# Yongda1/Ab-initio-Flexible-Gaussian-Basis-Neural-Network-Quantum-Monte-Carlo

Hardware: AMD Instinct MI355X
Metric: walker·steps/sec + local-energy evals/sec, N2 14e⁻ 4096 walkers, 1/2/4/8 MI355X (higher is better)
Workload: dtype f32

## Files before the change

### ab-initio-flexible-gaussian-basis-neural-network-quantum-monte-carlo_amd/csrc/quad_small.h

```cpp
#pragma once
#include "walker_rev.h"

namespace aq {

template <typename T> __device__ __forceinline__ T row16_sum(T x) {
  x += dpp<0x128>(x);
  x += dpp<0x124>(x);
  x += dpp<0x122>(x);
  x += dpp<0x121>(x);
  return x;
}
template <typename T> __device__ __forceinline__ T row_class4_sum(T x) {
  x += dpp<0x124>(x);
  x += dpp<0x128>(x);
  return x;
}

template <int N> struct QSlot {
  static constexpr int SW = N <= 4 ? 16 : 32;
  static constexpr int NI = SW / 4;
  static constexpr int NSL = 64 / SW;
};
template <int SW, typename T> __device__ __forceinline__ T slot_sum(T x) {
  x = row16_sum(x);
// ... 524 lines not shown
        if (acc && act) {
#pragma unroll
          for (int c = 0; c < 3; ++c) ((T*)ka.pos)[(size_t)conf * 3 * N + 3 * sl + c] = xn[c];
          if (ka.acc.count) atomicAdd(&ka.acc.count[conf], 1);
        }
      }
    } else if (sl < 3 * N) {
      xs[sl] = ((const T*)ka.pos)[(size_t)conf * 3 * N + sl];
    }
    wave_sync();
    {
      const int c = sl / NI, e = sl % NI;
      const int ee = e < N ? e : N - 1;
      const bool elive = e < N, ev = c == 3;
      ElecOut<T, A> eo;
      electron_stage<T, N, A>(P, xs + ee * 3, ee, c, eo);
      T* Wl = Wc + WC::loc + 16 * (ev ? 0 : c) + ee;
#pragma unroll
      for (int col = 0; col < N; ++col) {
        PJ<T> sy = P[Ly::wy + col] * eo.yst[0];
#pragma unroll
        for (int m = 1; m < NYW; ++m) sy = sy + P[Ly::wy + m * N + col] * eo.yst[m];
        const PJ<T> yt = eo.env * sy;
        lv[col] = yt.d1;
        if (elive && ev) {
          Yv[e * N + col] = yt.v;
          if (act) Wc[WC::yv + e * N + col] = yt.v;
        }
        if (elive && !ev && act) Wl[col * 48] = yt.d1;
      }
#pragma unroll
      for (int m = 0; m < D0; ++m) {
        lv[N + m] = eo.hf[m].d1;
        if (elive && ev) {
          hl[e * D0 + m] = eo.hf[m].v;
          if (act) Wc[WC::h0 + e * D0 + m] = eo.hf[m].v;
        }
        if (elive && !ev && act) Wl[(N + m) * 48] = eo.hf[m].d1;
      }
      if (elive && ev) {
        jsum = eo.jae.v;
        if (act) Wc[WC::jaev + e] = eo.jae.v;
      }
      if (elive && !ev) {
        jd1w = eo.jae.d1;
        if (act) Wc[WC::jaed + 16 * c + e] = jd1w;
      }
    }
    T jl = T(0);
#pragma unroll
    for (int it0 = 0; it0 < N * N; it0 += SW) {
      const int it = it0 + sl;
      const bool pl = it < N * N;
      const int k = pl ? it / N : 0, i = pl ? it - (it / N) * N : 0;
      const bool diag = k == i;
      T d[3];
#pragma unroll
      for (int c = 0; c < 3; ++c) d[c] = xs[i * 3 + c] - xs[k * 3 + c];
      const T r2 = d[0] * d[0] + d[1] * d[1] + d[2] * d[2];
      const T r = f_sqrt(diag ? T(1) : r2);
      T pp[4] = {diag ? T(0) : r, diag ? T(0) : d[0], diag ? T(0) : d[1], diag ? T(0) : d[2]};
      if (pl && k < i) {
        const T cusp = P[Ly::jee_c + k * N + i], al = P[Ly::jee_a + k * N + i];
        jl += f_div(cusp * r, al * r + T(1));
      }
      if (pl) {
#pragma unroll
        for (int f = 0; f < 4; ++f) S[it * 12 + f] = pp[f];
      }
#pragma unroll
      for (int j = 0; j < 2; ++j) {
        const cptr<T> dw = P + (j == 0 ? Ly::dbl_w0 : Ly::dbl_w1);
        const cptr<T> db = P + (j == 0 ? Ly::dbl_b0 : Ly::dbl_b1);
        T q[4];
#pragma unroll
        for (int o = 0; o < 4; ++o) {
          T z = db[o];
#pragma unroll
          for (int m = 0; m < 4; ++m) z += pp[m] * dw[m * 4 + o];
          q[o] = f_tanh(z);
        }
        if (pl && !diag && act) {
#pragma unroll
          for (int o = 0; o < 4; ++o) Wc[WC::pt + (k * N + i) * 8 + j * 4 + o] = q[o];
        }
#pragma unroll
        for (int o = 0; o < 4; ++o) {
          pp[o] = (pp[o] + q[o]) * RSQ2;
          if (pl) S[it * 12 + (j + 1) * 4 + o] = pp[o];
        }
      }
    }
    {
      jsum += jl;
      const T jee = slot_sum<SW>(jl);
      if (sl == 0 && act) Wc[WC::jee] = jee;
    }
    wave_sync();
    for (int t = sl; t < 24 * N; t += SW) {
      const int f = t & 3, ci = (t >> 2) % N, lg = (t >> 2) / N;
      const int l = lg >> 1, G = lg & 1;
      const int k0 = G ? nup : 0, k1 = G ? N : nup;
      T acc = T(0);
      for (int k = k0; k < k1; ++k) acc += S[(k * N + ci) * 12 + l * 4 + f];
      const T v = acc * (G ? ginv1 : ginv0);
      g2[((l * 2 + G) * N + ci) * 4 + f] = v;
      if (act) Wc[WC::g2 + ((l * 2 + G) * N + ci) * 4 + f] = v;
    }
    wave_sync();
  } else {
  jsum = quad_stage_load<T, N, A, SW>((const T*)ka.pos + (size_t)pb * 3 * N, Wc, Eq, pi, sl, xs, sm + SQ::xo, Yv,
                                      hl, g2);
  wave_sync();

  {
    const int part = sl / NI, o = sl % NI;
    const int os = o < N ? o : N - 1;
    const T* xp = (part & 1) ? sm + SQ::xo : xs + pi * 3;
    T d[3];
#pragma unroll
    for (int c = 0; c < 3; ++c) d[c] = part < 2 ? xs[os * 3 + c] - xp[c] : xp[c] - xs[os * 3 + c];
    T v[3][4];
    pair_values<T, N, A>(d, P, v);
    T dv[3][4];
#pragma unroll
    for (int l = 0; l < 3; ++l)
#pragma unroll
      for (int f = 0; f < 4; ++f) dv[l][f] = v[l][f] - dpp<0x100 + NI>(v[l][f]);
    if (part < 2 && o < N && o != pi) {
      const T cusp = P[Ly::jee_c + pi * N + o], al = P[Ly::jee_a + pi * N + o];
      const T je = f_div(cusp * v[0][0], al * v[0][0] + T(1));
      jsum += part == 0 ? je : -je;
    }
    if (part == 0 && o < N && o != pi) {
      const int Gp = pi >= nup ? 1 : 0;
      const T gw = Gp ? ginv1 : ginv0;
#pragma unroll
      for (int l = 0; l < 3; ++l)
#pragma unroll
        for (int f = 0; f < 4; ++f) g2[((l * 2 + Gp) * N + o) * 4 + f] += dv[l][f] * gw;
    }
    if (part == 2) {
#pragma unroll
      for (int l = 0; l < 3; ++l)
#pragma unroll
        for (int f = 0; f < 4; ++f) S[o * 12 + l * 4 + f] = dv[l][f];
    }
  }
  wave_sync();
#pragma unroll
  for (int t0 = 0; t0 < 24; t0 += SW) {
    const int t = t0 + sl;
    if (t < 24) {
      const int l = t >> 3, G = (t >> 2) & 1, f = t & 3;
      const int k0 = G ? nup : 0, k1 = G ? N : nup;
      T acc = T(0);
      for (int k = k0; k < k1; ++k)
        if (k != pi) acc += S[k * 12 + l * 4 + f];
      g2[((l * 2 + G) * N + pi) * 4 + f] += acc * (G ? ginv1 : ginv0);
    }
  }
  wave_sync();
  }

  const int fi = sl >> 2, ff = sl & 3;
  const bool ilive = fi < N;
  const int ic = ilive ? fi : N - 1;
// ... 492 lines not shown
```

### ab-initio-flexible-gaussian-basis-neural-network-quantum-monte-carlo_amd/csrc/walker_rev.h

```cpp
#pragma once
#include "jets.h"
#include "layout.h"
#include "walker_kernel.h"
#include "gj.h"
#include "electron.h"

namespace aq {

#ifdef AQ_PHASE_PROF
static __device__ unsigned long long aq_phase_cycles[32];
#define AQ_PH(k)                                                                         \
  do {                                                                                   \
    const unsigned long long t_ = __builtin_readcyclecounter();                          \
    if (lane == 0) atomicAdd(&aq_phase_cycles[(ka.proposal ? 16 : 0) + (k)], t_ - t_ph); \
    t_ph = t_;                                                                           \
  } while (0)
#elif defined(AQ_PHASE_MARK)
#define AQ_PH(k) asm volatile(";AQMARK " #k)
#elif defined(AQ_STOP_AFTER)
#define AQ_PH(k)                                                                     \
  do {                                                                               \
    if constexpr (PROP && (k) == AQ_STOP_AFTER) {                                    \
      if (ka.logabs) ((T*)ka.logabs)[conf * 64 + lane] = sm[lane] + sm[lane + 1024]; \
      return;                                                                        \
    }                                                                                \
  } while (0)
#else
#define AQ_PH(k) \
  do {           \
  } while (0)
#endif

#ifdef AQ_ABLATE
#define AQ_ABL(b) (isprop && (ka.ablate & (b)))
#else
#define AQ_ABL(b) false
#endif

#ifndef AQ_NO_FWD_REG
constexpr bool kFwdReg = true;
#else
constexpr bool kFwdReg = false;
#endif
template <typename T, int N, int A, bool FWDREG = false, bool COMPACT = false>
struct SmemRev {
  static constexpr int D0 = 4 * A;
  static constexpr int DFM = 3 * D0 + 8;
  static constexpr int QM = DFM / 4;
  static constexpr int hl_n = N * D0 + N * 4;
  static constexpr int cmax(int a, int b) { return a > b ? a : b; }
  static constexpr int xs = 0;
  static constexpr int hl = 48;
  static constexpr int hbar = hl;
  static constexpr int QL = (3 * 4 + 8) / 4;
  static constexpr int cq = hl + hl_n;
  static constexpr int sv = cq + (FWDREG ? 0 : N * QM + 2 * N * QL);
  static constexpr int cqo(int l, int i) { return l == 0 ? i * QM : N * QM + ((l - 1) * N + i) * QL; }
  static constexpr int g2 = sv + (FWDREG ? 0 : 3 * N * 4);
  static constexpr int yv = g2 + 3 * 2 * N * 4;
  static constexpr int ybar = yv;
  static constexpr int R = yv + N * N;
  static constexpr int ph = R;
  static constexpr int mx = COMPACT ? R : R + N * N * 2;
  static constexpr int dbar = R;
  static constexpr int R_n = COMPACT ? cmax(cmax(2 * N * N, 3 * N * N), 4 + 32 * 12)
                                     : cmax(cmax(4 * N * N, 3 * N * N), 4 + 64 * 12);
  static constexpr int pv = g2;
  static constexpr int RW = (N + 3) / 4;
  static constexpr int st = ((g2 + 3 * N + 2 + 3) / 4) * 4;
  static constexpr int zr = st + (4 * RW * 4 * 4 + (int)sizeof(T) - 1) / (int)sizeof(T);
  static_assert(zr + 4 <= g2 + 3 * 2 * N * 4, "slot table outside the g2 region");
  static constexpr int jdo = R + R_n;
  static constexpr int end = jdo + (FWDREG ? 64 : 0);
  static constexpr int bytes = ((end * (int)sizeof(T)) + 15) & ~15;
  static constexpr int hoff(int l) { return l == 0 ? 0 : N * D0; }
};

template <int N, int A>
struct WCache {
  static constexpr int D0 = 4 * A;
  static constexpr int yv = 0;
  static constexpr int h0 = yv + N * N;
  static constexpr int loc = h0 + N * D0;
  static constexpr int jaev = loc + (N + D0) * 48;
  static constexpr int jaed = jaev + N;
  static constexpr int g2 = jaed + 48;
  static constexpr int jee = g2 + 3 * 2 * N * 4;
  static constexpr int pv = jee + 1;
  static constexpr int pt = ((pv + 3 * N + 2 + 3) / 4) * 4;
  static constexpr int size = ((pt + 8 * N * N + 63) / 64) * 64;
};
template <int N, int A>
struct ECache {
  static constexpr int D0 = 4 * A;
  static constexpr int yv = 0;
  static constexpr int h0 = N;
  static constexpr int yd = N + D0;
  static constexpr int hd = yd + 3 * N;
  static constexpr int jv = hd + 3 * D0;
  static constexpr int jd = jv + 1;
  static constexpr int xp = jd + 3;
  static constexpr int size = ((xp + 3 + 15) / 16) * 16;
};

template <typename T, int N, int A>
__device__ __forceinline__ void pair_values(const T d[3], cptr<T> P, T out[3][4]) {
  using Ly = Lay<N, A>;
  const T RSQ2 = T(0.70710678118654752);
  T p[4];
  p[0] = f_sqrt(d[0] * d[0] + d[1] * d[1] + d[2] * d[2]);
#pragma unroll
  for (int c = 0; c < 3; ++c) p[1 + c] = d[c];
#pragma unroll
  for (int f = 0; f < 4; ++f) out[0][f] = p[f];
#pragma unroll
  for (int j = 0; j < 2; ++j) {
    const cptr<T> dw = P + (j == 0 ? Ly::dbl_w0 : Ly::dbl_w1);
    const cptr<T> db = P + (j == 0 ? Ly::dbl_b0 : Ly::dbl_b1);
    T q[4];
#pragma unroll
    for (int o = 0; o < 4; ++o) {
      T s = db[o];
#pragma unroll
      for (int m = 0; m < 4; ++m) s += p[m] * dw[m * 4 + o];
      q[o] = f_tanh(s);
    }
#pragma unroll
    for (int o = 0; o < 4; ++o) {
      p[o] = (p[o] + q[o]) * RSQ2;
      out[j + 1][o] = p[o];
    }
  }
}

template <typename T> __device__ __forceinline__ T class4_sum(T x) {
  x += dpp<0x124>(x);
  x += dpp<0x128>(x);
#ifdef AQ_PERMLANE_SUM
  if constexpr (sizeof(T) == 4) {
    const auto a = __builtin_amdgcn_permlane16_swap(__float_as_uint(x), __float_as_uint(x), false, false);
    x = __uint_as_float(a[0]) + __uint_as_float(a[1]);
    const auto b = __builtin_amdgcn_permlane32_swap(__float_as_uint(x), __float_as_uint(x), false, false);
    return __uint_as_float(b[0]) + __uint_as_float(b[1]);
  }
#endif
  x += __shfl_xor(x, 16);
  x += __shfl_xor(x, 32);
  return x;
}
template <int M, typename T> __device__ __forceinline__ T quad_bcast(T x) {
  return dpp<M | (M << 2) | (M << 4) | (M << 6)>(x);
}

template <typename T, int NV, int NU>
__device__ __forceinline__ void ld_use(cptr<T> p, T* out) {
  static_assert(NU <= NV, "record");
  if constexpr (sizeof(T) == 4) {
    typedef float f4 __attribute__((ext_vector_type(4)));
    typedef float f2 __attribute__((ext_vector_type(2)));
    const __attribute__((address_space(4))) f4* q = (const __attribute__((address_space(4))) f4*)p;
#pragma unroll
    for (int j = 0; j < NU / 4; ++j) {
      const f4 v = q[j];
      out[4 * j] = v.x;
      out[4 * j + 1] = v.y;
      out[4 * j + 2] = v.z;
      out[4 * j + 3] = v.w;
    }
    constexpr int B = NU / 4 * 4, R = NU % 4;
    if constexpr (R >= 2) {
      const f2 v = *(const __attribute__((address_space(4))) f2*)(p + B);
      out[B] = v.x;
      out[B + 1] = v.y;
    }
    if constexpr (R == 1 || R == 3) out[B + R - 1] = p[B + R - 1];
#pragma unroll
    for (int k = NU; k < NV; ++k) out[k] = T(0);
  } else {
#pragma unroll
    for (int k = 0; k < NV; ++k) out[k] = k < NU ? p[k] : T(0);
  }
}

template <typename T, int NV>
__device__ __forceinline__ void ld_vec(cptr<T> p, T* out) {
  if constexpr (sizeof(T) == 4) {
    typedef float f4 __attribute__((ext_vector_type(4)));
    const __attribute__((address_space(4))) f4* q = (const __attribute__((address_space(4))) f4*)p;
#pragma unroll
    for (int j = 0; j < NV / 4; ++j) {
      const f4 v = q[j];
      out[4 * j] = v.x;
      out[4 * j + 1] = v.y;
      out[4 * j + 2] = v.z;
      out[4 * j + 3] = v.w;
    }
  } else {
    typedef double d2 __attribute__((ext_vector_type(2)));
    const __attribute__((address_space(4))) d2* q = (const __attribute__((address_space(4))) d2*)p;
#pragma unroll
    for (int j = 0; j < NV / 2; ++j) {
      const d2 v = q[j];
      out[2 * j] = v.x;
      out[2 * j + 1] = v.y;
    }
  }
}
#ifndef AQ_NO_XLANE
constexpr bool kXLane = true;
#else
constexpr bool kXLane = false;
#endif

__device__ __forceinline__ void wave_sync() {
  __builtin_amdgcn_fence(__ATOMIC_RELEASE, "wavefront");
// ... 145 lines not shown
  T* E = (T*)ka.ecache + (size_t)q0 * EC::size;
#pragma unroll
  for (int col = 0; col < N; ++col) {
    PJ<T> sy = P[Ly::wy + col] * eo.yst[0];
#pragma unroll
    for (int m = 1; m < NYW; ++m) sy = sy + P[Ly::wy + m * N + col] * eo.yst[m];
    E[EC::yv + col] = (eo.env * sy).v;
  }
#pragma unroll
  for (int m = 0; m < D0; ++m) E[EC::h0 + m] = eo.hf[m].v;
  E[EC::jv] = eo.jae.v;
#pragma unroll
  for (int c = 0; c < 3; ++c) E[EC::xp + c] = xp[c];
}

#ifndef AQ_PROP_WAVES
#define AQ_PROP_WAVES 5
#endif
#ifndef AQ_PREP_WAVES
#define AQ_PREP_WAVES 4
#endif
template <typename T, int N, int A, bool PREP, bool PROP, bool PW7 = false> struct RevWaves {
  static constexpr int value = PW7 ? 7 : (PREP ? (sizeof(T) == 4 ? AQ_PREP_WAVES : 2) : ((sizeof(T) == 4 && N == 14 && A == 2) ? (PROP ? AQ_PROP_WAVES : 4) : 1));
};

#ifndef AQ_PROP_WPB
#define AQ_PROP_WPB 2
#endif
#ifndef AQ_WALK_WPB
#define AQ_WALK_WPB 1
#endif
template <typename T, bool PROP, bool PREP = false> struct RevWpb {
  static constexpr int value = sizeof(T) != 4 ? 1 : (PROP ? AQ_PROP_WPB : (PREP ? 1 : AQ_WALK_WPB));
};
#ifdef AQ_WAVE_SYNC
#define AQ_SYNC() wave_sync()
#else
#define AQ_SYNC()                                   \
  do {                                              \
    if constexpr (WPB > 1) wave_sync();             \
    else __syncthreads();                           \
  } while (0)
#endif

template <typename T, int N, int A>
__device__ __forceinline__ void b3_pair_adjoint(cptr<T> P, const T* xs, const T* g2b, T* dbar, int nup, int k, int i,
                                                bool may_fresh, bool fresh, const T* tcache, T cusp, T al) {
  using Ly = Lay<N, A>;
  const T RSQ2 = T(0.70710678118654752);
  cptr<T> Pq = P;
  asm volatile("" : "+s"(Pq));
  const int G = k >= nup ? 1 : 0;
  T d[3];
#pragma unroll
  for (int c = 0; c < 3; ++c) d[c] = xs[i * 3 + c] - xs[k * 3 + c];
  const T r = f_sqrt(d[0] * d[0] + d[1] * d[1] + d[2] * d[2]);
  T p0[4] = {r, d[0], d[1], d[2]};
  T t1[4], t2[4];
#pragma unroll
  for (int o = 0; o < 4; ++o) {
    t1[o] = tcache ? tcache[o] : T(0);
    t2[o] = tcache ? tcache[4 + o] : T(0);
  }
  if (may_fresh) {
    T f1[4], p1[4], f2[4];
#pragma unroll
    for (int o = 0; o < 4; ++o) {
      T s = Pq[Ly::dbl_b0 + o];
#pragma unroll
      for (int m = 0; m < 4; ++m) s += p0[m] * Pq[Ly::dbl_w0 + m * 4 + o];
      f1[o] = f_tanh(s);
    }
#pragma unroll
    for (int o = 0; o < 4; ++o) p1[o] = (p0[o] + f1[o]) * RSQ2;
#pragma unroll
    for (int o = 0; o < 4; ++o) {
      T s = Pq[Ly::dbl_b1 + o];
#pragma unroll
      for (int m = 0; m < 4; ++m) s += p1[m] * Pq[Ly::dbl_w1 + m * 4 + o];
      f2[o] = f_tanh(s);
    }
#pragma unroll
    for (int o = 0; o < 4; ++o) {
      t1[o] = fresh ? f1[o] : t1[o];
      t2[o] = fresh ? f2[o] : t2[o];
    }
  }
  T pb2[4], pb1[4], pb0[4];
#pragma unroll
  for (int f = 0; f < 4; ++f) pb2[f] = g2b[((2 * 2 + G) * N + i) * 4 + f];
  T z2[4];
#pragma unroll
  for (int o = 0; o < 4; ++o) z2[o] = pb2[o] * RSQ2 * (T(1) - t2[o] * t2[o]);
#pragma unroll
  for (int m = 0; m < 4; ++m) {
    T s = g2b[((1 * 2 + G) * N + i) * 4 + m] + pb2[m] * RSQ2;
#pragma unroll
    for (int o = 0; o < 4; ++o) s += z2[o] * Pq[Ly::dbl_w1 + m * 4 + o];
    pb1[m] = s;
  }
  T z1[4];
#pragma unroll
  for (int o = 0; o < 4; ++o) z1[o] = pb1[o] * RSQ2 * (T(1) - t1[o] * t1[o]);
#pragma unroll
  for (int m = 0; m < 4; ++m) {
    T s = g2b[((0 * 2 + G) * N + i) * 4 + m] + pb1[m] * RSQ2;
#pragma unroll
    for (int o = 0; o < 4; ++o) s += z1[o] * Pq[Ly::dbl_w0 + m * 4 + o];
    pb0[m] = s;
  }
  T rb = pb0[0];
  {
    const T den = al * r + T(1);
    rb += and_zero(k < i, cusp * f_rcp(den * den));
  }
  const T ir = f_rcp(r);
#pragma unroll
  for (int c = 0; c < 3; ++c) dbar[(k * N + i) * 3 + c] = pb0[1 + c] + rb * d[c] * ir;
}

template <typename T, int N>
__device__ __forceinline__ void walker_draws(const __attribute__((address_space(4))) KArgs* kl, int conf, int lane) {
  if (kl->dg1 && lane < N) {
    const uint32_t t = (uint32_t)(conf * N + lane);
    const uint64_t seed = kl->seed, step = kl->step;
    float a[3], b[3], c[4];
    philox_normal3f(seed, step, t, 0u, a);
    philox_normal3f(seed, step, t, 1u, b);
    philox_u4(seed, step, t, 2u, c);
#pragma unroll
    for (int k = 0; k < 3; ++k) {
      ((T*)kl->dg1)[(size_t)t * 3 + k] = (T)a[k];
      ((T*)kl->dg2)[(size_t)t * 3 + k] = (T)b[k];
    }
    ((T*)kl->du)[t] = (T)(c[0] - 5.9604644775390625e-08f);
  }
}

template <typename T, int N, int A, bool PREP = false, bool PROP = false, bool PW7 = false, bool PH = false,
          bool SPL = false>
__global__ __attribute__((amdgpu_flat_work_group_size(1, 64 * (SPL ? 2 : RevWpb<T, PROP, PREP>::value)))) __attribute__((amdgpu_waves_per_eu(RevWaves<T, N, A, PREP, PROP, PW7>::value))) void
k_walker_rev(KArgs ka) {
  static_assert(!PW7 || (PROP && !PREP), "PW7 is a proposal instantiation");
  static_assert(!PH || PREP, "PH is an adjoint-pass instantiation");
  static_assert(!SPL || (!PROP && !PREP), "SPL is a walker-launch instantiation");
  using Ly = Lay<N, A>;
  constexpr bool fwd_reg = PROP && kFwdReg;
  constexpr bool compact = PROP && PW7 && fwd_reg;
  constexpr bool xlane = PROP && kXLane;
  using SM = SmemRev<T, N, A, fwd_reg, compact>;
  using LCc = LapCache<N, A>;
  constexpr int D0 = SM::D0;
  constexpr int WPB = SPL ? 2 : RevWpb<T, PROP, PREP>::value;
  const cptr<T> P = param_ptr<T>(ka.prm);
  extern __shared__ __attribute__((aligned(16))) unsigned char smem_raw[];
  const int wv = WPB > 1 ? __builtin_amdgcn_readfirstlane((int)(threadIdx.x >> 6)) : 0;
  T* sm = (T*)(smem_raw + (SPL ? 0 : wv) * SM::bytes);
  T* xs = sm + SM::xs;

  const bool isprop = PROP ? true : (ka.proposal != 0);
  const int conf = SPL ? xcd_major(blockIdx.x, gridDim.x) : xcd_major(blockIdx.x, gridDim.x) * WPB + wv;
  if (WPB > 1 && conf >= ka.nconf) return;
  const int lane = WPB > 1 ? (int)(threadIdx.x & 63) : (int)threadIdx.x;
  const int lc = lane >> 4;
  const int er = lane & 15;
  const int le = er < N ? er : N - 1;
  const bool val = (lc == 3);
  const bool live = er < N;
  const bool dir = (lc < 3) && live;
  const int nup = ka.nup;
  const T tstep = (T)ka.tstep;
  const T RSQ2 = T(0.70710678118654752);
  const T ginv0 = T(1) / T(nup), ginv1 = T(1) / T(N - nup);
  const int* rowsrc = ka.rowsrc;
#ifdef AQ_PHASE_PROF
  unsigned long long t_ph = __builtin_readcyclecounter();
#endif

  int pb = conf, pi = -1;
  if (isprop) {
    const int mper = ka.mper ? ka.mper : N, mdiv = ka.mdiv ? ka.mdiv : 1;
    pb = conf / mper;
    pi = (conf - pb * mper) / mdiv;
  }
  const T te_walk = (!PROP && isprop && !ka.xnew) ? taueff_wave<T>(ka.taueff, ka.tacc, 0, ka.tstep, ka.tpart) : T(0);
  if (SPL && wv != 0) {
  } else if (!PREP && !isprop && ka.acc.lpn) {
    const T te1 = taueff_wave<T>(ka.acc.taueff, ka.acc.tacc, 0, ka.acc.tstep, ka.acc.tpart);
    const T te2 = taueff_wave<T>(ka.acc.taueff, ka.acc.tacc, 1, ka.acc.tstep, ka.acc.tpart);
    if (lane < N) {
      T xn[3];
      const bool acc = accept_one<T, N>(ka.acc, (const T*)ka.pos, conf, lane, xn, te1, te2);
#pragma unroll
      for (int c = 0; c < 3; ++c) xs[3 * lane + c] = xn[c];
      if (acc) {
#pragma unroll
        for (int c = 0; c < 3; ++c) ((T*)ka.pos)[(size_t)conf * 3 * N + 3 * lane + c] = xn[c];
        if (ka.acc.count) atomicAdd(&ka.acc.count[conf], 1);
      }
    }
  } else if (!PROP && lane < 3 * N) {
    T x = ((const T*)ka.pos)[(size_t)pb * 3 * N + lane];
    if (isprop && lane / 3 == pi) {
      sm[SM::R + (lane - 3 * pi)] = x;
      if (ka.xnew) {
        x = ((const T*)ka.xnew)[(size_t)conf * 3 + (lane - 3 * pi)];
      } else {
        const T z = ((const T*)ka.gauss1)[(size_t)pb * 3 * N + lane];
        const T ge = ((const T*)ka.pgrad)[(size_t)pb * 3 * N + lane] * te_walk;
        x = x + (ge * tstep + f_sqrt(tstep) * z);
      }
    }
    xs[lane] = x;
  }
  if constexpr (SPL) __syncthreads();
  else if constexpr (!PROP) AQ_SYNC();

  AQ_PH(0);
  using WC = WCache<N, A>;
  using EC = ECache<N, A>;
  const bool reuse = !PREP && PROP;
#ifndef AQ_NO_F1_GLDS
  constexpr bool f1_glds = PROP;
#else
  constexpr bool f1_glds = false;
#endif
  const bool wfix = !PREP && !PROP && !isprop && ka.pvok != 0;
  T* Wc = (T*)ka.wcache + (size_t)(reuse ? pb : conf) * WC::size;
  T* Lw = PREP ? (T*)ka.lapcache + (size_t)conf * LCc::size : nullptr;
  const T* Eq = reuse ? (const T*)ka.ecache + (size_t)conf * EC::size : nullptr;
  T* Yv = sm + SM::yv;
  T* g2 = sm + SM::g2;
  T jv = T(0), jd1 = T(0), jve = T(0);
  T jsum_p = T(0);
  T pvr = T(0);
  int rsl = 0;
  T jvp = T(0);
  auto f2_pair_values = [&](T cusp, T al) {
    T* S = sm + SM::R + 4;
    const T* xo = sm + SM::R;
    const int o = lane & 15, part = lane >> 4;
    const int os = o < N ? o : N - 1;
    const T* xp = (part & 1) ? xo : xs + pi * 3;
    T d[3];
#pragma unroll
    for (int c = 0; c < 3; ++c) d[c] = (part < 2) ? xs[os * 3 + c] - xp[c] : xp[c] - xs[os * 3 + c];
    T v[3][4];
    pair_values<T, N, A>(d, P, v);
    if constexpr (compact) {
#pragma unroll
      for (int l = 0; l < 3; ++l)
#pragma unroll
        for (int f = 0; f < 4; ++f) {
          const T w = __shfl_down(v[l][f], 16);
          if ((part & 1) == 0) S[(16 * (part >> 1) + o) * 12 + l * 4 + f] = v[l][f] - w;
        }
    } else {
#pragma unroll
    for (int l = 0; l < 3; ++l)
#pragma unroll
      for (int f = 0; f < 4; ++f) S[lane * 12 + l * 4 + f] = v[l][f];
    }
    if (part < 2 && o < N && o != pi) {
      if constexpr (!PROP) {
        cusp = P[Ly::jee_c + pi * N + o];
        al = P[Ly::jee_a + pi * N + o];
      }
      const T je = f_div(cusp * v[0][0], al * v[0][0] + T(1));
      jvp += part == 0 ? je : -je;
    }
  };
  auto jee_params = [&](T& cusp, T& al) {
    const int os = (lane & 15) < N ? (lane & 15) : N - 1;
    cusp = P[Ly::jee_c + pi * N + os];
    al = P[Ly::jee_a + pi * N + os];
  };
  if (reuse) {
    constexpr int NY = (N * N + 63) / 64, NHh = (N * D0 + 63) / 64, NG = (3 * 2 * N * 4 + 63) / 64;
    T ry[NY], rh[NHh], rg[NG];
    T eyv = T(0), eh0 = T(0);
    if constexpr (f1_glds) {
      lds_dma<T>(Yv, Wc + WC::yv, N * N, lane);
      lds_dma<T>(sm + SM::hl, Wc + WC::h0, N * D0, lane);
      lds_dma<T>(g2, Wc + WC::g2, 3 * 2 * N * 4, lane);
      eyv = Eq[EC::yv + (lane < N ? lane : N - 1)];
      eh0 = Eq[EC::h0 + (lane < D0 ? lane : D0 - 1)];
    }
    const bool mvl = lane < 3 * N && lane / 3 == pi;
    T x0 = T(0), xm = T(0), jc = T(0), ja = T(0);
    if constexpr (PROP) {
      const int l3 = lane < 3 * N ? lane : 3 * N - 1;
      x0 = ((const T*)ka.pos)[(size_t)pb * 3 * N + l3];
      xm = Eq[EC::xp + (mvl ? lane - 3 * pi : 0)];
      jee_params(jc, ja);
      rsl = rowsrc[lane < N ? lane : N - 1];
    }
    if constexpr (!f1_glds) {
#pragma unroll
    for (int t = 0; t < NY; ++t) {
      const unsigned idx = lane + 64 * t;
      const unsigned ix = idx < N * N ? idx : N * N - 1;
      const unsigned r = ix / N;
      const T a = Wc[WC::yv + ix], b = Eq[EC::yv + (ix - r * N)];
      ry[t] = ((int)r == pi) ? b : a;
    }
#pragma unroll
    for (int t = 0; t < NHh; ++t) {
      const unsigned idx = lane + 64 * t;
      const unsigned ix = idx < N * D0 ? idx : N * D0 - 1;
      const unsigned e = ix / D0;
      const T a = Wc[WC::h0 + ix], b = Eq[EC::h0 + (ix - e * D0)];
      rh[t] = ((int)e == pi) ? b : a;
    }
#pragma unroll
    for (int t = 0; t < NG; ++t) {
      const int idx = lane + 64 * t;
      rg[t] = Wc[WC::g2 + (idx < 3 * 2 * N * 4 ? idx : 3 * 2 * N * 4 - 1)];
    }
    }
    {
      if constexpr (PROP) {
        const T* js = (er == pi) ? Eq + EC::jv : Wc + WC::jaev + le;
        jv = and_zero(val && live, *js);
        const T* ds = (le == pi) ? Eq + EC::jd + (lc < 3 ? lc : 0) : Wc + WC::jaed + (lane < 48 ? lane : 47);
        jd1 = and_zero(dir, *ds);
        jve = and_zero(lane == 0, Wc[WC::jee]);
      } else {
        const T a = Wc[WC::jaev + le], b = Eq[EC::jv];
        jv = (val && live) ? ((er == pi) ? b : a) : T(0);
        const T a1 = Wc[WC::jaed + (lane < 48 ? lane : 47)], b1 = Eq[EC::jd + (lc < 3 ? lc : 0)];
        jd1 = dir ? ((le == pi) ? b1 : a1) : T(0);
// ... 75 lines not shown
#pragma unroll
        for (int l = 0; l < 3; ++l)
#pragma unroll
          for (int f = 0; f < 4; ++f)
            g2[((l * 2 + Gp) * N + lane) * 4 + f] +=
                (compact ? S[lane * 12 + l * 4 + f] : S[lane * 12 + l * 4 + f] - S[(16 + lane) * 12 + l * 4 + f]) * gw;
      }
    } else if (lane < 40) {
      const int t = lane - 16;
      const int l = t >> 3, G = (t >> 2) & 1, f = t & 3;
      const int k0 = G ? nup : 0, k1 = G ? N : nup;
      T acc = T(0);
#pragma unroll
      for (int k = 0; k < N; ++k) {
        const T dv = compact ? S[(16 + k) * 12 + l * 4 + f] : S[(32 + k) * 12 + l * 4 + f] - S[(48 + k) * 12 + l * 4 + f];
        acc += (k >= k0 && k < k1 && k != pi) ? dv : T(0);
      }
      g2[((l * 2 + G) * N + pi) * 4 + f] += acc * (G ? ginv1 : ginv0);
    }
  } else if (!reuse && (!SPL || wv == 1)) {
    {
      const int i = lane >> 2, kq = lane & 3;
      const bool icol = i < N;
      const int ii = icol ? i : N - 1;
      T acc[3][2][4];
  #pragma unroll
      for (int l = 0; l < 3; ++l)
  #pragma unroll
        for (int G = 0; G < 2; ++G)
  #pragma unroll
          for (int f = 0; f < 4; ++f) acc[l][G][f] = T(0);
      constexpr int NT = (N + 3) / 4;
      T jcp[NT], jap[NT];
  #pragma unroll
      for (int t = 0; t < NT; ++t) {
        const int kk = kq + 4 * t < N ? kq + 4 * t : N - 1;
        jcp[t] = P[Ly::jee_c + kk * N + ii];
        jap[t] = P[Ly::jee_a + kk * N + ii];
      }
      T dwv[2][16], dbv[2][4];
  #pragma unroll
      for (int j = 0; j < 2; ++j) {
        const cptr<T> dw = P + (j == 0 ? Ly::dbl_w0 : Ly::dbl_w1);
        const cptr<T> db = P + (j == 0 ? Ly::dbl_b0 : Ly::dbl_b1);
  #pragma unroll
        for (int k = 0; k < 16; ++k) dwv[j][k] = dw[k];
  #pragma unroll
        for (int k = 0; k < 4; ++k) dbv[j][k] = db[k];
      }
  #pragma unroll
      for (int t = 0; t < NT; ++t) {
        const int k = kq + 4 * t;
        if (k < N) {
          const bool diag = (k == ii);
          T d[3];
  #pragma unroll
          for (int c = 0; c < 3; ++c) d[c] = xs[ii * 3 + c] - xs[k * 3 + c];
          const T r2 = d[0] * d[0] + d[1] * d[1] + d[2] * d[2];
          const T r = f_sqrt(diag ? T(1) : r2);
          T p[4] = {diag ? T(0) : r, diag ? T(0) : d[0], diag ? T(0) : d[1], diag ? T(0) : d[2]};
          if (icol && k < ii) {
            const T cusp = jcp[t], al = jap[t];
            jve += f_div(cusp * r, al * r + T(1));
          }
          const bool G1 = k >= nup;
  #pragma unroll
          for (int f = 0; f < 4; ++f) {
            acc[0][0][f] += G1 ? T(0) : p[f];
            acc[0][1][f] += G1 ? p[f] : T(0);
          }
  #pragma unroll
          for (int j = 0; j < 2; ++j) {
            T q[4];
  #pragma unroll
            for (int o = 0; o < 4; ++o) {
              T s = dbv[j][o];
  #pragma unroll
              for (int m = 0; m < 4; ++m) s += p[m] * dwv[j][m * 4 + o];
              q[o] = f_tanh(s);
            }
            if (!PREP && !isprop && icol && !diag) {
              T* tp = Wc + WC::pt + (k * N + ii) * 8 + j * 4;
#pragma unroll
              for (int o = 0; o < 4; ++o) tp[o] = q[o];
            }
            if (PREP && icol) {
              T* tp = Lw + LCc::pt + (k * N + ii) * LCc::pt_n + j * 4;
#pragma unroll
              for (int o = 0; o < 4; ++o) tp[o] = q[o];
            }
  #pragma unroll
            for (int o = 0; o < 4; ++o) {
              p[o] = (p[o] + q[o]) * RSQ2;
              acc[j + 1][0][o] += G1 ? T(0) : p[o];
              acc[j + 1][1][o] += G1 ? p[o] : T(0);
            }
          }
        }
      }
  #pragma unroll
      for (int l = 0; l < 3; ++l)
  #pragma unroll
        for (int G = 0; G < 2; ++G)
  #pragma unroll
          for (int f = 0; f < 4; ++f) {
            T v = acc[l][G][f];
            v += dpp<0xB1>(v);
            v += dpp<0x4E>(v);
            if (icol && kq == 0) g2[((l * 2 + G) * N + i) * 4 + f] = v * (G ? ginv1 : ginv0);
          }
    }
  }
  AQ_SYNC();
  if (!PREP && !isprop && (!SPL || wv == 1)) {
    for (int idx = lane; idx < 3 * 2 * N * 4; idx += 64) Wc[WC::g2 + idx] = g2[idx];
    const T je = wave_sum(jve);
    if (lane == 0) Wc[WC::jee] = je;
    if (SPL) sm[SM::R + lane] = jve;
  }
  if constexpr (SPL) {
    __syncthreads();
    if (wv != 0) {
      walker_draws<T, N>(late_args(), conf, lane);
      if (ka.wcache) {
        __syncthreads();
        __builtin_amdgcn_fence(__ATOMIC_RELEASE, "workgroup");
        __builtin_amdgcn_fence(__ATOMIC_ACQUIRE, "workgroup");
        constexpr int NPR = N * (N - 1);
        for (int it = 64 + lane; it < NPR; it += 128) {
          const int k = it / (N - 1);
          const int jj = it - k * (N - 1);
          const int i = jj + (jj >= k ? 1 : 0);
          b3_pair_adjoint<T, N, A>(P, xs, sm + SM::g2, sm + SM::dbar, nup, k, i, false, false,
                                   Wc + WC::pt + (k * N + i) * 8, P[Ly::jee_c + k * N + i], P[Ly::jee_a + k * N + i]);
        }
        __syncthreads();
      }
      return;
    }
    jve = sm[SM::R + lane];
  }

  AQ_PH(2);
  T* hl = sm + SM::hl;
  T* cqv = sm + SM::cq;
  T* sv = sm + SM::sv;
  T cqr[3][2], svr[3];
  const int fi = lane >> 2, ff = lane & 3;
  const bool ilive = fi < N;
  const int ic = ilive ? fi : N - 1;
  const bool inG1 = ic >= nup;
  T hreg = T(0);
#ifndef AQ_NO_PHI_MFMA
  constexpr bool phi_mfma = PROP && sizeof(T) == 4 && (N + 3) / 4 == 4 && NH == 4;
#else
  constexpr bool phi_mfma = false;
#endif
  using V2o = typename Pair<T>::type;
  V2o ow[8], obs[2];
  T owm[4];
  auto orb_load = [&]() {
    const int cl = (lane & 15) < N ? (lane & 15) : N - 1;
    const cptr<T> wcol = P + 2 * cl;
    if constexpr (phi_mfma) {
      const int fq = lane >> 4;
#pragma unroll
      for (int s = 0; s < 2; ++s) {
// ... 769 lines not shown
        for (int c = 0; c < NC; ++c) {
          s0[c] += dpp<0xB1>(s0[c]);
          s0[c] += dpp<0x4E>(s0[c]);
#pragma unroll
          for (int j = 0; j < 2; ++j)
#pragma unroll
            for (int f = 0; f < 4; ++f) {
              s1[j][c][f] += dpp<0xB1>(s1[j][c][f]);
              s1[j][c][f] += dpp<0x4E>(s1[j][c][f]);
            }
        }
        if (ilv && kq < NC) {
          const int c = C0 + kq;
          const T cnt = T(k1 - k0 - ((ii >= k0 && ii < k1) ? 1 : 0));
          T* o0 = Lw + LCc::sd + ((G * N + ii) * 3 + c) * 4;
          o0[0] = (NC == 1 || kq == 0) ? s0[0] : s0[NC - 1];
#pragma unroll
          for (int f = 1; f < 4; ++f) o0[f] = (f - 1 == c) ? cnt : T(0);
#pragma unroll
          for (int j = 0; j < 2; ++j) {
            T* oj = Lw + (j + 1) * LCc::layer_n + LCc::sd + ((G * N + ii) * 3 + c) * 4;
#pragma unroll
            for (int f = 0; f < 4; ++f) oj[f] = (NC == 1 || kq == 0) ? s1[j][0][f] : s1[j][NC - 1][f];
          }
        }
      }
    };
    pair_pass(std::integral_constant<int, 0>{}, std::integral_constant<int, 2>{});
    pair_pass(std::integral_constant<int, 2>{}, std::integral_constant<int, 1>{});
    pcurv = T(2) * wave_sum(pcurv);
    const T lpsi = logdet + wave_sum(jv + jve);
    if (lane == 0) {
      Lw[LCc::scal] = pcurv;
      if (ka.logabs) ((T*)ka.logabs)[conf] = lpsi;
      if (ka.phase) ((T*)ka.phase)[conf] = f_atan2(phi, phr);
    }
    return;
  }

  const int c4 = lc < 3 ? lc : 0;
  T lv[N + D0];
  auto lv_load = [&]() {
    const bool mov = reuse && le == pi;
    const T* la = mov ? Eq + EC::yd + c4 * N : Wc + WC::loc + (lane < 48 ? lane : 47);
    const T* lb = mov ? Eq + EC::hd + c4 * D0 : Wc + WC::loc + N * 48 + (lane < 48 ? lane : 47);
    const int st = mov ? 1 : 48;
#pragma unroll
    for (int m = 0; m < N; ++m) lv[m] = la[m * st];
#pragma unroll
    for (int m = 0; m < D0; ++m) lv[N + m] = lb[m * st];
  };
#ifndef AQ_LV_AT
#define AQ_LV_AT 0
#endif
  constexpr int lv_at = (reuse && PROP) ? AQ_LV_AT : 0;
  if (lv_at == 0) lv_load();
  AQ_PH(6);
  T* dbar = sm + SM::dbar;
  auto pair_adjoint = [&](int k, int i, bool may_fresh, bool fresh, const T* tcache, T cusp, T al) {
    b3_pair_adjoint<T, N, A>(P, xs, g2b, dbar, nup, k, i, may_fresh, fresh, tcache, cusp, al);
  };
  constexpr int NPR = N * (N - 1);
  if (reuse && !AQ_ABL(32)) {
    constexpr int M = 2 * (N - 1);
    constexpr int NIT = (NPR + 63) / 64;
    T tc[NIT][8], jc[NIT], ja[NIT];
    int pk[NIT], pi2[NIT];
#pragma unroll
    for (int u = 0; u < NIT; ++u) {
      const unsigned code = pair_tab<N>.v[pi][lane + 64 * u];
      const int k = code & 15, i = (code >> 4) & 15;
      pk[u] = k;
      pi2[u] = i;
      jc[u] = P[Ly::jee_c + k * N + i];
      ja[u] = P[Ly::jee_a + k * N + i];
    }
#pragma unroll
    for (int u = 0; u < NIT; ++u) {
      const int k = pk[u], i = pi2[u];
      const T* tp = Wc + WC::pt + (k * N + i) * 8;
#pragma unroll
      for (int o = 0; o < 8; ++o) tc[u][o] = tp[o];
    }
#pragma unroll
    for (int u = 0; u < NIT; ++u) {
      const int it = lane + 64 * u;
      if (it < NPR) pair_adjoint(pk[u], pi2[u], u == 0, u == 0 && it < M, tc[u], jc[u], ja[u]);
      if (lv_at == u + 1) lv_load();
    }
  } else if (!reuse) {
    if (!PREP && !isprop && ka.wcache) {
      if constexpr (SPL) __syncthreads();
      __builtin_amdgcn_fence(__ATOMIC_RELEASE, "workgroup");
      __builtin_amdgcn_fence(__ATOMIC_ACQUIRE, "workgroup");
      for (int it = lane; it < NPR; it += SPL ? 128 : 64) {
        const int k = it / (N - 1);
        const int jj = it - k * (N - 1);
        const int i = jj + (jj >= k ? 1 : 0);
        pair_adjoint(k, i, false, false, Wc + WC::pt + (k * N + i) * 8, P[Ly::jee_c + k * N + i], P[Ly::jee_a + k * N + i]);
      }
      if constexpr (SPL) __syncthreads();
    } else {
      for (int it = lane; it < NPR; it += 64) {
        const int k = it / (N - 1);
        const int jj = it - k * (N - 1);
        const int i = jj + (jj >= k ? 1 : 0);
        pair_adjoint(k, i, true, true, nullptr, P[Ly::jee_c + k * N + i], P[Ly::jee_a + k * N + i]);
      }
    }
  }
  AQ_SYNC();

  AQ_PH(7);
  T g = fwd_reg ? sm[SM::jdo + lane] : jd1;
  if (!AQ_ABL(64)) {
    T ga = T(0), gb = T(0), gc = T(0);
#pragma unroll
    for (int k = 0; k < N; ++k) {
      const T dk = dbar[(k * N + le) * 3 + c4] - dbar[(le * N + k) * 3 + c4];
      if (k & 1) ga += (k == le) ? T(0) : dk;
      else g += (k == le) ? T(0) : dk;
    }
#pragma unroll
    for (int col = 0; col < N; ++col) {
      if (col & 1) gc = f_fma(ybar[le * N + col], lv[col], gc);
      else gb = f_fma(ybar[le * N + col], lv[col], gb);
    }
#pragma unroll
    for (int m = 0; m < D0; ++m) {
      if (m & 1) gc = f_fma(hbar[le * D0 + m], lv[N + m], gc);
      else gb = f_fma(hbar[le * D0 + m], lv[N + m], gb);
    }
    g = (g + ga) + (gb + gc);
  }

  AQ_PH(8);
  const T gd = dir ? g : T(0);
  const T sumsq = wave_sum(gd * gd);
  const T lpsi = logdet + (fwd_reg ? jsum_p : wave_sum(jv + jve));
  const auto* kl = late_args();
  if (kl->grad && dir) ((T*)kl->grad)[(size_t)conf * 3 * N + 3 * le + lc] = g;
  if (kl->gown && dir && le == pi) ((T*)kl->gown)[(size_t)conf * 3 + lc] = g;
  if (lane == 0) {
    if (kl->logabs) ((T*)kl->logabs)[conf] = lpsi;
    if (kl->phase) ((T*)kl->phase)[conf] = f_atan2(phi, phr);
    if (kl->sumsq) ((T*)kl->sumsq)[conf] = sumsq;
    if (kl->tacc) tacc_add(kl->tacc, isprop ? 1 : 0, conf, (double)sumsq);
  }
  if constexpr (!PREP && !SPL) {
    if (!isprop) walker_draws<T, N>(kl, conf, lane);
  }
  AQ_PH(9);
}

}
```

Baseline: 14.39 million.

## Cache tanh-derivative factors and hand over moved-pair tanh values via LDS

Stores the precomputed backprop factor RSQ2*(1-t^2) in the pair cache instead of the raw tanh value, so the adjoint pass only needs a multiply. It also writes the freshly computed pair tanh values for the moved electron into a new shared-memory handover region. The reverse pass then reads them from there instead of recomputing pair_values for the first iteration. This trades extra LDS footprint and stores for fewer tanh evaluations and fewer FLOPs in the reverse pass.

```diff
diff --git a/ab-initio-flexible-gaussian-basis-neural-network-quantum-monte-carlo_amd/csrc/quad_small.h b/ab-initio-flexible-gaussian-basis-neural-network-quantum-monte-carlo_amd/csrc/quad_small.h
--- a/ab-initio-flexible-gaussian-basis-neural-network-quantum-monte-carlo_amd/csrc/quad_small.h
+++ b/ab-initio-flexible-gaussian-basis-neural-network-quantum-monte-carlo_amd/csrc/quad_small.h
@@ -630,7 +630,7 @@
         }
         if (pl && !diag && act) {
 #pragma unroll
-          for (int o = 0; o < 4; ++o) Wc[WC::pt + (k * N + i) * 8 + j * 4 + o] = q[o];
+          for (int o = 0; o < 4; ++o) Wc[WC::pt + (k * N + i) * 8 + j * 4 + o] = pt_rec(q[o]);
         }
 #pragma unroll
         for (int o = 0; o < 4; ++o) {
diff --git a/ab-initio-flexible-gaussian-basis-neural-network-quantum-monte-carlo_amd/csrc/walker_rev.h b/ab-initio-flexible-gaussian-basis-neural-network-quantum-monte-carlo_amd/csrc/walker_rev.h
--- a/ab-initio-flexible-gaussian-basis-neural-network-quantum-monte-carlo_amd/csrc/walker_rev.h
+++ b/ab-initio-flexible-gaussian-basis-neural-network-quantum-monte-carlo_amd/csrc/walker_rev.h
@@ -42,6 +42,19 @@
 #else
 constexpr bool kFwdReg = false;
 #endif
+#ifndef AQ_NO_B3_HANDOVER
+constexpr bool kB3Handover = true;
+#else
+constexpr bool kB3Handover = false;
+#endif
+#ifndef AQ_PT_TANH
+constexpr bool kPtFactor = true;
+#else
+constexpr bool kPtFactor = false;
+#endif
+template <typename T> __device__ __forceinline__ T pt_rec(T t) {
+  return kPtFactor ? T(0.70710678118654752) * (T(1) - t * t) : t;
+}
 template <typename T, int N, int A, bool FWDREG = false, bool COMPACT = false>
 struct SmemRev {
   static constexpr int D0 = 4 * A;
@@ -71,7 +84,9 @@
   static constexpr int zr = st + (4 * RW * 4 * 4 + (int)sizeof(T) - 1) / (int)sizeof(T);
   static_assert(zr + 4 <= g2 + 3 * 2 * N * 4, "slot table outside the g2 region");
   static constexpr int jdo = R + R_n;
-  static constexpr int end = jdo + (FWDREG ? 64 : 0);
+  static constexpr bool hand = FWDREG && kB3Handover;
+  static constexpr int th = (jdo + (FWDREG ? 64 : 0) + 3) / 4 * 4;
+  static constexpr int end = hand ? th + 2 * 2 * 16 * 4 : jdo + (FWDREG ? 64 : 0);
   static constexpr int bytes = ((end * (int)sizeof(T)) + 15) & ~15;
   static constexpr int hoff(int l) { return l == 0 ? 0 : N * D0; }
 };
@@ -104,7 +119,7 @@
 };
 
 template <typename T, int N, int A>
-__device__ __forceinline__ void pair_values(const T d[3], cptr<T> P, T out[3][4]) {
+__device__ __forceinline__ void pair_values(const T d[3], cptr<T> P, T out[3][4], T tq[2][4]) {
   using Ly = Lay<N, A>;
   const T RSQ2 = T(0.70710678118654752);
   T p[4];
@@ -127,10 +142,16 @@
     }
 #pragma unroll
     for (int o = 0; o < 4; ++o) {
+      tq[j][o] = q[o];
       p[o] = (p[o] + q[o]) * RSQ2;
       out[j + 1][o] = p[o];
     }
   }
+}
+template <typename T, int N, int A>
+__device__ __forceinline__ void pair_values(const T d[3], cptr<T> P, T out[3][4]) {
+  T tq[2][4];
+  pair_values<T, N, A>(d, P, out, tq);
 }
 
 template <typename T> __device__ __forceinline__ T class4_sum(T x) {
@@ -442,8 +463,8 @@
     }
 #pragma unroll
     for (int o = 0; o < 4; ++o) {
-      t1[o] = fresh ? f1[o] : t1[o];
-      t2[o] = fresh ? f2[o] : t2[o];
+      t1[o] = fresh ? pt_rec(f1[o]) : t1[o];
+      t2[o] = fresh ? pt_rec(f2[o]) : t2[o];
     }
   }
   T pb2[4], pb1[4], pb0[4];
@@ -451,7 +472,7 @@
   for (int f = 0; f < 4; ++f) pb2[f] = g2b[((2 * 2 + G) * N + i) * 4 + f];
   T z2[4];
 #pragma unroll
-  for (int o = 0; o < 4; ++o) z2[o] = pb2[o] * RSQ2 * (T(1) - t2[o] * t2[o]);
+  for (int o = 0; o < 4; ++o) z2[o] = kPtFactor ? pb2[o] * t2[o] : pb2[o] * RSQ2 * (T(1) - t2[o] * t2[o]);
 #pragma unroll
   for (int m = 0; m < 4; ++m) {
     T s = g2b[((1 * 2 + G) * N + i) * 4 + m] + pb2[m] * RSQ2;
@@ -461,7 +482,7 @@
   }
   T z1[4];
 #pragma unroll
-  for (int o = 0; o < 4; ++o) z1[o] = pb1[o] * RSQ2 * (T(1) - t1[o] * t1[o]);
+  for (int o = 0; o < 4; ++o) z1[o] = kPtFactor ? pb1[o] * t1[o] : pb1[o] * RSQ2 * (T(1) - t1[o] * t1[o]);
 #pragma unroll
   for (int m = 0; m < 4; ++m) {
     T s = g2b[((0 * 2 + G) * N + i) * 4 + m] + pb1[m] * RSQ2;
@@ -605,8 +626,18 @@
     T d[3];
 #pragma unroll
     for (int c = 0; c < 3; ++c) d[c] = (part < 2) ? xs[os * 3 + c] - xp[c] : xp[c] - xs[os * 3 + c];
-    T v[3][4];
-    pair_values<T, N, A>(d, P, v);
+    T v[3][4], tq[2][4];
+    pair_values<T, N, A>(d, P, v, tq);
+    if constexpr (SM::hand) {
+      if ((part & 1) == 0 && o < N && o != pi) {
+#pragma unroll
+        for (int j = 0; j < 2; ++j) {
+          T* th = (T*)__builtin_assume_aligned(sm + SM::th + (((part >> 1) * 2 + j) * 16 + o) * 4, 16);
+#pragma unroll
+          for (int f = 0; f < 4; ++f) th[f] = pt_rec(tq[j][f]);
+        }
+      }
+    }
     if constexpr (compact) {
 #pragma unroll
       for (int l = 0; l < 3; ++l)
@@ -848,7 +879,7 @@
             if (!PREP && !isprop && icol && !diag) {
               T* tp = Wc + WC::pt + (k * N + ii) * 8 + j * 4;
 #pragma unroll
-              for (int o = 0; o < 4; ++o) tp[o] = q[o];
+              for (int o = 0; o < 4; ++o) tp[o] = pt_rec(q[o]);
             }
             if (PREP && icol) {
               T* tp = Lw + LCc::pt + (k * N + ii) * LCc::pt_n + j * 4;
@@ -1784,10 +1815,23 @@
 #pragma unroll
       for (int o = 0; o < 8; ++o) tc[u][o] = tp[o];
     }
+    if constexpr (SM::hand) {
+      const int hp = pk[0] == pi ? 0 : 1, ho = pk[0] == pi ? pi2[0] : pk[0];
+      T hv[8];
+#pragma unroll
+      for (int j = 0; j < 2; ++j) {
+        const T* th = (const T*)__builtin_assume_aligned(sm + SM::th + ((hp * 2 + j) * 16 + ho) * 4, 16);
+#pragma unroll
+        for (int f = 0; f < 4; ++f) hv[j * 4 + f] = th[f];
+      }
+#pragma unroll
+      for (int o = 0; o < 8; ++o) tc[0][o] = lane < M ? hv[o] : tc[0][o];
+    }
 #pragma unroll
     for (int u = 0; u < NIT; ++u) {
       const int it = lane + 64 * u;
-      if (it < NPR) pair_adjoint(pk[u], pi2[u], u == 0, u == 0 && it < M, tc[u], jc[u], ja[u]);
+      const bool rc = !SM::hand && u == 0;
+      if (it < NPR) pair_adjoint(pk[u], pi2[u], rc, rc && it < M, tc[u], jc[u], ja[u]);
       if (lv_at == u + 1) lv_load();
     }
   } else if (!reuse) {
```

Result: faster. 14.74 million (median of 6 runs) (+2.5%).
